# google-research/simclr

Measured on AMD Instinct MI355X. Metric: images/sec (whole node), ResNet-50 1x SimCLR pretraining step @224px, higher is better.
Workload: dtype f32; 1 GPU; ResNet-50 1x, 224x224, 2 views/image, per-GPU batch 512, global batch 512, NT-Xent T=0.1 + linear-eval head + LARS, global BN, dp1; global_batch=512, parallelism=dp1

## Files before the change

### simclr_amd/csrc/conv.hip

```cpp
#include "common.h"
#include <stdlib.h>
#include <string.h>
#include <mutex>
#include <type_traits>

namespace {

enum { MODE_FWD = 0, MODE_DGRAD = 1 };

struct ConvP {
  const void* x;
  const void* w;
  void* y;
  float* stats;
  int V, IH, IW, IC, OH, OW, N, KH, KW, stride, pad;
  int pixpitch;
  int M, K;
  int nslot, accumulate;
  int m_tiles, n_tiles;
  int cs, py, px, cls_h, cls_w;
  int ntaps;
  int taps[9];
  unsigned long long tap_w, dy_w, dx_w;
  const void* bn_x;
// ... 364 lines not shown
#pragma unroll
        for (int o = 1; o < 16; o <<= 1) { s += __shfl_xor(s, o, 64); ss += __shfl_xor(ss, o, 64); }
        if (fl == 0) {
          const int nl = wn * 64 + ni * 16 + g * 4 + r;
          red[(wm * BN + nl) * 2] = s;
          red[(wm * BN + nl) * 2 + 1] = ss;
        }
      }
    }
    __syncthreads();
    if (tid < BN && n0 + tid < p.N) {
      float s = 0.f, ss = 0.f;
#pragma unroll
      for (int w = 0; w < WM; ++w) { s += red[(w * BN + tid) * 2]; ss += red[(w * BN + tid) * 2 + 1]; }
      float* st = p.stats + (long long)(mt % p.nslot) * 2 * p.N;
      atomicAdd(st + n0 + tid, s);
      atomicAdd(st + p.N + n0 + tid, ss);
    }
    __syncthreads();
  }

  if (LDS_EPI) {
    constexpr int PITCH = BN * 2 + 8;
    constexpr int LPR = BN * 2 / 8;
    unsigned char* Cs = smem;
    long long* rowoff = (long long*)(smem + BM * PITCH);
    if (tid < BM) rowoff[tid] = row_offset(m0 + tid);
#pragma unroll
    for (int ni = 0; ni < NI; ++ni) {
      const int nl = wn * 64 + ni * 16 + g * 4;
#pragma unroll
      for (int mi = 0; mi < MI; ++mi) {
        const int ml = wm * (MI * 16) + mi * 16 + fl;
        u32x2 pk;
        pk[0] = pack_bf16x2(acc[ni][mi][0], acc[ni][mi][1]);
        pk[1] = pack_bf16x2(acc[ni][mi][2], acc[ni][mi][3]);
        *(u32x2*)(Cs + ml * PITCH + nl * 2) = pk;
      }
    }
    __syncthreads();
    const int c8 = tid % LPR;
    const int ncol = n0 + c8 * 4;
#pragma unroll 4
    for (int r = tid / LPR; r < BM; r += 256 / LPR) {
      const long long off = rowoff[r];
      if (off >= 0 && ncol < p.N) {
        u32x2 v = *(const u32x2*)(Cs + r * PITCH + c8 * 8);
        uint16_t* dst = (uint16_t*)Y + off + ncol;
        if (p.accumulate) {
          const u32x2 o = *(const u32x2*)dst;
          v[0] = pack_bf16x2(__uint_as_float(v[0] << 16) + __uint_as_float(o[0] << 16),
                             __uint_as_float(v[0] & 0xffff0000u) + __uint_as_float(o[0] & 0xffff0000u));
          v[1] = pack_bf16x2(__uint_as_float(v[1] << 16) + __uint_as_float(o[1] << 16),
                             __uint_as_float(v[1] & 0xffff0000u) + __uint_as_float(o[1] & 0xffff0000u));
        }
        *(u32x2*)dst = v;
      }
    }
  } else {
#pragma unroll
    for (int mi = 0; mi < MI; ++mi) {
      const long long off = row_offset(m0 + wm * (MI * 16) + mi * 16 + fl);
#pragma unroll
      for (int ni = 0; ni < NI; ++ni) {
        const int n = n0 + wn * 64 + ni * 16 + g * 4;
        if (off >= 0 && n < p.N) {
          T* dst = Y + off + n;
          float v[4] = {acc[ni][mi][0], acc[ni][mi][1], acc[ni][mi][2], acc[ni][mi][3]};
          if (p.accumulate) {
#pragma unroll
            for (int r = 0; r < 4; ++r) v[r] += Elem<T>::ld(dst + r);
          }
          *(float4*)dst = make_float4(v[0], v[1], v[2], v[3]);
        }
      }
    }
  }
}

#ifndef SIMCLR_BN64_WPE
#define SIMCLR_BN64_WPE 3
#endif
template <typename T, int MODE, int BM, int BN, int NW, int STAGES, bool STATS, bool BNEPI, bool EXT = false,
          bool WIN = false, bool FAPPLY = false, int SPL = 0, bool TAIL = false, bool PSB = false, int FAS = 0, int EPS = 0, bool PSX = false>
__global__ __launch_bounds__(NW * 64, (NW == 8 || STAGES == 3) ? 1 : (BN == 64 && (sizeof(T) == 2 || SPL == 13 || (SPL == 3 && PSB))) ? SIMCLR_BN64_WPE : 2) void conv_igemm_persistent(const ConvP p) {
  static_assert(EPS == 0 || (BNEPI && EPS <= 4 && (sizeof(T) == 2 || (MODE == MODE_DGRAD && SPL == 3 && PSB && PSX && !EXT))), "EPS specialises the BNEPI epilogue");
  const int bnm = EPS ? (((EPS - 1) >> 1) ? 4 : 2) : p.bn_mode;
  const bool accu = EPS ? ((EPS - 1) & 1) != 0 : p.accumulate != 0;
  static_assert(FAS == 0 || FAPPLY, "FAS specialises the FAPPLY epilogue");
  const bool fa_res = FAS ? true : p.bn_x != nullptr;
  const bool fa_rbn = FAS ? FAS == 2 : p.bn_mean != nullptr;
  const bool fa_relu = FAS ? true : p.bn_mode != 0;
  const bool fa_mask = FAS ? true : p.bn_mask != nullptr;
  const bool fa_n32 = FAS ? true : (p.N & 31) == 0;
  static_assert(!PSB || ((SPL == 3 || SPL == 13) && sizeof(T) == 4), "pre-split weights: fp32 storage, three terms");
  static_assert(!PSX || ((SPL == 3 || SPL == 13) && sizeof(T) == 4), "pre-split gathered operand: fp32 storage, three terms");
  static_assert(SPL != 13 || PSB, "split-fp16 terms need the pre-split (scaled) weight planes");
  static_assert(!WIN || (STAGES == 2 && !EXT && NW == 4 && BM == 128 && !FAPPLY && (sizeof(T) == 2 || ((SPL == 3 || SPL == 13) && PSB))),
                "halo-window variant: 2 stages; bf16, or fp32 storage with three terms and pre-split weights");
  static_assert(!FAPPLY || (MODE == MODE_FWD && !STATS && !BNEPI && !EXT), "fused BN-apply epilogue: forward, no statistics");
  static_assert(SPL == 0 || sizeof(T) == 4, "split-bf16 terms: fp32 storage only");
  constexpr bool WPS = WIN && sizeof(T) == 4 && !PSX && (SPL == 3 || SPL == 13);
  constexpr int EPC = Elem<T>::EPC;
  constexpr int BK = 8 * EPC;
  constexpr int WN = BN / 64;
  constexpr int WM = NW / WN;
  constexpr int MI = BM / WM / 16;
  constexpr int NI = 4;
  constexpr int AJ = BM / (8 * NW);
  constexpr int BJ = BN / (8 * NW);
  static_assert(AJ >= 1 && BJ >= 1 && MI >= 1, "tile / wave configuration");
  extern __shared__ __attribute__((aligned(16))) unsigned char smem[];
  constexpr int STG = (BM + BN) * 8;
  u32x4* As = (u32x4*)smem;
  u32x4* Bs = As + BM * 8;
  u32x4* Wn = (u32x4*)smem;
  u32x4* Bw = (u32x4*)(smem + (WIN ? p.win_bytes : 0));
  float* bnp = WIN ? (float*)(Bw + 2 * BN * 8)
                   : (float*)(As + STAGES * STG);
  long long* rowoff = (long long*)(bnp + (4 + (EXT ? 1 : 0)) * BN);
  const int zrow = WIN ? (int)(((unsigned char*)(rowoff + BM) - smem) >> 7) : 0;
  constexpr bool WSUM = BM == 256;
  float2* wred = (float2*)(rowoff + BM);
  constexpr bool LDS_EPI = sizeof(T) == 2;
  constexpr int NTH = NW * 64;
  constexpr int CPR = BN / 8;
  constexpr int RPP = NTH / CPR;
  constexpr bool ROWSTATS = STATS && LDS_EPI && (BNEPI || BM == 256);
  constexpr int EH = (LDS_EPI && BM * BN * 2 > STG * 16) ? 2 : 1;
  constexpr int BMH = BM / EH;
  static_assert(!LDS_EPI || (BMH * BN * 2 <= STG * 16), "C (half) tile must fit in one stage");
  static_assert(EH == 1 || (WM % EH == 0 && !WIN), "half-tile epilogue: whole waves per half");
  typedef __attribute__((address_space(1))) const void* gptr_t;
  typedef __attribute__((address_space(3))) void* lptr_t;

  const int tid = threadIdx.x, lane = tid & 63;
  const int wave = __builtin_amdgcn_readfirstlane(tid >> 6);
  const int g = lane >> 4, fl = lane & 15;
  const int wm = wave / WN, wn = wave % WN;
  const T* __restrict__ X = (const T*)p.x;
  const T* __restrict__ Wt = (const T*)p.w;
  T* __restrict__ Y = (T*)p.y;
  const int cls_hw = p.cls_h * p.cls_w;

  const int xcd = blockIdx.x & 7, l = blockIdx.x >> 3;
  const int nt = l % p.n_tiles;
  const int mslots = gridDim.x / p.n_tiles;
  const int mslot = (l / p.n_tiles) * 8 + xcd;
  const int n0 = nt * BN;
  const int count = (TAIL && p.rem_parts >= 2) ? p.rem_full : ((mslot < p.m_tiles) ? (p.m_tiles - mslot + mslots - 1) / mslots : 0);
  const bool has_part = TAIL && p.rem_parts >= 2 && mslot < p.rem_tiles * p.rem_parts;
  auto part_tile = [&]() __attribute__((always_inline)) { return p.rem_full * mslots + mslot / p.rem_parts; };
  auto part_index = [&]() __attribute__((always_inline)) { return mslot % p.rem_parts; };
  const int kpt = p.IC / BK;
  const int kpt2 = EXT ? p.ic2 / BK : 0;
  const int KT = p.ntaps * kpt + kpt2;
  const int kmain = p.KH * p.KW * p.IC;
  const T* __restrict__ X2 = (const T*)p.x2;

  const int kc = (lane & 7) ^ (lane >> 3);
  const bool flat = WIN || (p.KH == 1 && p.KW == 1 && p.stride == 1 && p.pad == 0 && p.cs == 1 &&
                            p.IH == p.OH && p.IW == p.OW);
  int a_ry[AJ], a_rx[AJ];
  int a_m[AJ];
  const T* a_rb[AJ];
  bool a_ok[AJ];
  const T* a_tp[AJ];
// ... 61 lines not shown
      __builtin_amdgcn_global_load_lds((gptr_t)src, (lptr_t)(b_dst + j * 1024), 16, 0, 0);
    }
  };

  if (BNEPI || EXT || FAPPLY) {
    for (int i = tid; i < BN; i += NW * 64) {
      const int n = n0 + i;
      const bool ok = n < p.N;
      if (FAPPLY) {
        bnp[i] = ok ? p.bn_scale[n] : 0.f;
        bnp[BN + i] = ok ? p.bn_shift[n] : 0.f;
        bnp[2 * BN + i] = (ok && p.bn_mean) ? p.bn_mean[n] : 1.f;
        bnp[3 * BN + i] = (ok && p.bn_rstd) ? p.bn_rstd[n] : 0.f;
      }
      if (BNEPI) {
        bnp[i] = (ok && bnm == 2) ? p.bn_scale[n] : 0.f;
        bnp[BN + i] = (ok && bnm == 2) ? p.bn_shift[n] : 0.f;
        bnp[2 * BN + i] = (ok && p.bn_mean) ? p.bn_mean[n] : 0.f;
        bnp[3 * BN + i] = (ok && p.bn_rstd) ? p.bn_rstd[n] : 0.f;
      }
      if (EXT) bnp[4 * BN + i] = (ok && p.bias) ? p.bias[n] : 0.f;
    }
  }
  if (WSUM && STATS && LDS_EPI) {
    for (int i = lane; i < BN; i += 64) wred[wave * BN + i] = make_float2(0.f, 0.f);
  }
  const int e_cc = tid % CPR;
  float e_s[8], e_q[8];
#pragma unroll
  for (int e = 0; e < 8; ++e) { e_s[e] = 0.f; e_q[e] = 0.f; }
  float st_s[NI][4], st_q[NI][4];
  if (STATS) {
#pragma unroll
    for (int i = 0; i < NI; ++i)
#pragma unroll
      for (int r = 0; r < 4; ++r) { st_s[i][r] = 0.f; st_q[i][r] = 0.f; }
  }

  int it = 0, iti = 0, ici = 0, ibuf = 0, buf = 0;
  int issued = 0, consumed = 0;
  const int KU = WIN ? kpt : KT;
  auto part_begin = [&]() __attribute__((always_inline)) { return (part_index() * KU) / p.rem_parts; };
  auto part_end = [&]() __attribute__((always_inline)) { return ((part_index() + 1) * KU) / p.rem_parts; };
  const int part_units = has_part ? part_end() - part_begin() : 0;
  const int total = WIN ? (count * kpt + part_units) * 9 : count * KT + part_units;
  auto issue_next = [&]() __attribute__((always_inline)) {
    issue_tile(iti, ici, ibuf);
    ibuf = (ibuf + 1 == STAGES) ? 0 : ibuf + 1;
    ++issued;
    if (++ici == ((EXT && iti == p.ntaps) ? kpt2 : kpt)) {
      ici = 0;
      if (++iti == p.ntaps + ((EXT && kpt2 > 0) ? 1 : 0)) {
        iti = 0;
        ++it;
        if (it < count) setup_rows(mslot + it * mslots);
        else if (it == count && has_part) {
          setup_rows(part_tile());
          const int pka = part_begin();
          iti = pka / kpt; ici = pka - iti * kpt;
          if (EXT && iti > p.ntaps) { iti = p.ntaps; ici = pka - p.ntaps * kpt; }
        }
      }
      if (it < count + (has_part ? 1 : 0) && iti < p.ntaps) set_tap(iti);
    }
  };
  const int Wd = p.IW;
  int wti = 0, wci = (WIN && count == 0 && has_part) ? part_begin() : 0, wit = 0;
  auto issue_b = [&]() __attribute__((always_inline)) {
    const int k0 = (int)((p.tap_w >> (4 * wti)) & 15) * p.IC + wci * BK;
    unsigned char* b_dst = (unsigned char*)(Bw + ibuf * (BN * 8)) + wave * BJ * 1024;
#pragma unroll
    for (int j = 0; j < BJ; ++j) {
      const void* src = b_ok[j] ? (const void*)(b_src[j] + k0) : p.zero;
      __builtin_amdgcn_global_load_lds((gptr_t)src, (lptr_t)(b_dst + j * 1024), 16, 0, 0);
    }
    ibuf ^= 1;
    ++issued;
    if (++wti == 9) {
      wti = 0;
      if (++wci == kpt) { wci = 0; if (++wit == count && has_part) wci = part_begin(); }
    }
  };
  auto issue_win = [&](int m0w, int c) __attribute__((always_inline)) {
    for (int j = 0; j < p.win_j; ++j) {
      const int blk = wave * p.win_j + j;
      const long long pix = (long long)m0w - (Wd + 1) + 8 * blk + (lane >> 3);
      const void* src = (pix >= 0 && pix < p.M) ? (const void*)(X + pix * p.pixpitch + c * BK + kc * EPC) : p.zero;
      __builtin_amdgcn_global_load_lds((gptr_t)src, (lptr_t)(smem + blk * 1024), 16, 0, 0);
    }
  };
  if (WIN) {
    if (tid < 8) Wn[zrow * 8 + tid] = zero16();
    if (total > 0) issue_b();
  } else if (total > 0) {
    if (count > 0) {
      setup_rows(mslot);
      set_tap(0);
    } else {
      setup_rows(part_tile());
      const int pka = part_begin();
      iti = pka / kpt; ici = pka - iti * kpt;
      if (EXT && iti > p.ntaps) { iti = p.ntaps; ici = pka - p.ntaps * kpt; }
      if (iti < p.ntaps) set_tap(iti);
    }
#pragma unroll
    for (int sidx = 0; sidx < STAGES - 1; ++sidx)
      if (issued < total) issue_next();
  }
  for (int ct = 0; ct < count + (has_part ? 1 : 0); ++ct) {
    const bool part = ct == count;
    const int m0 = (part ? part_tile() : mslot + ct * mslots) * BM;
    const int kt0 = part ? part_begin() : 0, kt1 = part ? part_end() : KU;
    f32x4 acc[NI][MI];
#pragma unroll
    for (int i = 0; i < NI; ++i)
#pragma unroll
      for (int j = 0; j < MI; ++j) acc[i][j] = (f32x4){0.f, 0.f, 0.f, 0.f};
    if (WIN) {
      const int m0w = m0;
      int rb[MI];
      unsigned vm[MI];
#pragma unroll
      for (int i = 0; i < MI; ++i) {
        const int ml = wm * (MI * 16) + i * 16 + fl;
        rb[i] = ml + Wd + 1;
        const int m = m0w + ml;
        unsigned msk = 0;
        if (m < p.M) {
          const int q = m / Wd, x = m - q * Wd, y = q % p.IH;
          const unsigned cm = (x > 0 ? 1u : 0u) | 2u | (x < Wd - 1 ? 4u : 0u);
          msk = (y > 0 ? cm : 0u) | (cm << 3) | (y < p.IH - 1 ? cm << 6 : 0u);
        }
        vm[i] = msk;
      }
      auto win_rows = [&](int t, int zr, int* rr) __attribute__((always_inline)) {
        const int ody = (int)((p.dy_w >> (4 * t)) & 15) - 8 - (MODE == MODE_FWD ? p.pad : 0);
        const int odx = (int)((p.dx_w >> (4 * t)) & 15) - 8 - (MODE == MODE_FWD ? p.pad : 0);
        const int doff = ody * Wd + odx, vbit = (ody + 1) * 3 + (odx + 1);
#pragma unroll
        for (int i = 0; i < MI; ++i) rr[i] = ((vm[i] >> vbit) & 1u) ? rb[i] + doff : zr;
      };
      auto win_load = [&](const u32x4* Wc, const int* rr, const u32x4* Bt, int ks, u32x4* af, u32x4* bf) __attribute__((always_inline)) {
#pragma unroll
        for (int i = 0; i < MI; ++i) af[i] = Wc[rr[i] * 8 + ((ks * 4 + g) ^ (rr[i] & 7))];
#pragma unroll
        for (int i = 0; i < NI; ++i) {
          const int r = wn * 64 + i * 16 + fl;
          bf[i] = Bt[r * 8 + ((ks * 4 + g) ^ (r & 7))];
        }
      };
      auto win_mma = [&](const u32x4* af, const u32x4* bf) __attribute__((always_inline)) {
#pragma unroll
        for (int ni = 0; ni < NI; ++ni)
#pragma unroll
          for (int mi = 0; mi < MI; ++mi) acc[ni][mi] = MMA<T>::run(bf[ni], af[mi], acc[ni][mi]);
      };
      auto win_step = [&](const u32x4* Wc, int zr, const u32x4* Bt, int t) __attribute__((always_inline)) {
        int rr[MI];
        win_rows(t, zr, rr);
        if constexpr (sizeof(T) == 4) {
          mma_f32_chunks<NI, MI, false, SPL, PSB, PSX || WPS>(&acc[0][0],
              [&](int i, int ks) { const int r = wn * 64 + i * 16 + fl; return Bt[r * 8 + ((ks * 4 + g) ^ (r & 7))]; },
              [&](int i, int ks) { return Wc[rr[i] * 8 + ((ks * 4 + g) ^ (rr[i] & 7))]; });
        } else {
#pragma unroll
        for (int ks = 0; ks < 2; ++ks) {
          u32x4 af[MI], bf[NI];
          win_load(Wc, rr, Bt, ks, af, bf);
          win_mma(af, bf);
        }
        }
      };
      for (int c = kt0; c < kt1; ++c) {
        __syncthreads();
        issue_win(m0w, c);
        for (int t = 0; t < 9; ++t) {
          asm volatile("s_waitcnt vmcnt(0)" ::: "memory");
          __syncthreads();
          if (issued < total) issue_b();
          if constexpr (WPS) {
            if (t == 0) {
              const int nq = p.win_j * 32 * 4;
              for (int q = tid; q < nq; q += NW * 64) {
                const int row = q >> 2, gq = q & 3;
                u32x4* w0 = Wn + row * 8 + (gq ^ (row & 7));
                u32x4* w1 = Wn + row * 8 + ((4 + gq) ^ (row & 7));
                u32x4 hi, lo;
                if constexpr (SPL == 13) split_terms2_f16(*w0, *w1, hi, lo); else split_terms2(*w0, *w1, hi, lo);
                *w0 = hi; *w1 = lo;
              }
              __syncthreads();
            }
          }
          win_step(Wn, zrow, Bw + buf * (BN * 8), t);
          buf ^= 1;
          ++consumed;
        }
      }
    } else
    for (int kt = kt0; kt < kt1; ++kt) {
      if (STAGES == 3 && issued - consumed >= 2) asm volatile("s_waitcnt vmcnt(%0)" ::"n"(AJ + BJ) : "memory");
      else asm volatile("s_waitcnt vmcnt(0)" ::: "memory");
      if (STAGES == 3) {
        asm volatile("s_waitcnt lgkmcnt(0)" ::: "memory");
        __builtin_amdgcn_s_barrier();
      } else {
        __syncthreads();
      }
      if (issued < total) issue_next();
      if constexpr (sizeof(T) == 4) {
        if (!DIAG(1))
          mma_f32_chunks<NI, MI, false, SPL, PSB, PSX>(&acc[0][0],
              [&](int i, int ks) { const int r = wn * 64 + i * 16 + fl; return Bs[buf * STG + r * 8 + ((ks * 4 + g) ^ (r & 7))]; },
              [&](int i, int ks) { const int r = wm * (MI * 16) + i * 16 + fl; return As[buf * STG + r * 8 + ((ks * 4 + g) ^ (r & 7))]; });
      } else
      if (!DIAG(1))
#pragma unroll
      for (int ks = 0; ks < 2; ++ks) {
        constexpr int MH = MI > 4 ? 4 : MI;
        u32x4 bf[NI];
#pragma unroll
        for (int i = 0; i < NI; ++i) {
          const int r = wn * 64 + i * 16 + fl;
          bf[i] = Bs[buf * STG + r * 8 + ((ks * 4 + g) ^ (r & 7))];
        }
#pragma unroll
        for (int mh = 0; mh < MI; mh += MH) {
          u32x4 af[MH];
#pragma unroll
          for (int i = 0; i < MH; ++i) {
            const int r = wm * (MI * 16) + (mh + i) * 16 + fl;
            af[i] = As[buf * STG + r * 8 + ((ks * 4 + g) ^ (r & 7))];
          }
#pragma unroll
          for (int ni = 0; ni < NI; ++ni)
#pragma unroll
            for (int mi = 0; mi < MH; ++mi) acc[ni][mh + mi] = MMA<T>::run(bf[ni], af[mi], acc[ni][mh + mi]);
        }
      }
      buf = (buf + 1 == STAGES) ? 0 : buf + 1;
      ++consumed;
    }
    if (DIAG(4)) {
      if (acc[0][0][0] == 12345.678f) Y[0] = (T)0;
      continue;
    }
    if constexpr (SPL == 13) {
#pragma unroll
      for (int i = 0; i < NI; ++i)
#pragma unroll
        for (int j = 0; j < MI; ++j) acc[i][j] *= (1.0f / (float)(1 << F16_WSCALE_LOG2));
    }
    if (part) {
      const long long slot0 = ((long long)(mslot / p.rem_parts) * p.n_tiles + nt) * (p.rem_parts - 1);
      const int pj = part_index();
      constexpr int FR = NI * MI;
      if (pj != 0) {
        const __amdgpu_buffer_rsrc_t rp = __builtin_amdgcn_make_buffer_rsrc(
            (void*)((f32x4*)p.part_ws + (slot0 + pj - 1) * (long long)(FR * NTH)), 0, FR * NTH * 16, 0x00020000);
#pragma unroll
        for (int ni = 0; ni < NI; ++ni)
#pragma unroll
          for (int mi = 0; mi < MI; ++mi)
            __builtin_amdgcn_raw_buffer_store_b128(__builtin_bit_cast(u32x4, acc[ni][mi]), rp, tid * 16, (ni * MI + mi) * NTH * 16, 16);
// ... 1985 lines not shown
  const long long nchunks = e[2] * 8;
  const bool f16 = e[3] != 0;
  for (long long i = blockIdx.x * 256ll + threadIdx.x; i < nchunks; i += (long long)gridDim.x * 256ll) {
    const long long blk = i >> 3;
    const int c = (int)(i & 7), gq = c & 3;
    u32x4 c0 = *(const u32x4*)(src + blk * 32 + gq * 4), c1 = *(const u32x4*)(src + blk * 32 + 16 + gq * 4);
    u32x4 hi, lo;
    if (f16) {
#pragma unroll
      for (int q = 0; q < 4; ++q) { c0[q] = __float_as_uint(__uint_as_float(c0[q]) * f16_scale); c1[q] = __float_as_uint(__uint_as_float(c1[q]) * f16_scale); }
      split_terms2_f16(c0, c1, hi, lo);
    } else {
      split_terms2(c0, c1, hi, lo);
    }
    *(u32x4*)(dst + i * 4) = (c < 4) ? hi : lo;
  }
}

__global__ __launch_bounds__(256) void presplit_packed(const float4* __restrict__ src, u32x4* __restrict__ dst, long long npix) {
  for (long long i = blockIdx.x * 256ll + threadIdx.x; i < npix; i += (long long)gridDim.x * 256ll) {
    const float4 v = src[i];
    uint32_t h0, l0, h1, l1;
    split_pair<false>(v.x, v.y, h0, l0);
    split_pair<false>(v.z, v.w, h1, l1);
    dst[i] = (u32x4){h0, h1, l0, l1};
  }
}

__global__ void unpack_stem_dw(const float* __restrict__ src, float* __restrict__ dst, int KH, int KW,
                               int CI, int CO, int KWP, int accumulate) {
  const int total = KH * KW * CI * CO;
  for (int i = blockIdx.x * blockDim.x + threadIdx.x; i < total; i += gridDim.x * blockDim.x) {
    const int co = i % CO;
    const int ci = (i / CO) % CI;
    const int kw = (i / (CO * CI)) % KW;
    const int kh = i / (CO * CI * KW);
    const float v = src[(long long)((kh * KWP + kw) * 4 + ci) * CO + co];
    dst[i] = accumulate ? dst[i] + v : v;
  }
}

static int g_f32_terms_fwd = 0, g_f32_terms_bwd = 0;
static bool valid_terms(int t, bool fwd) { return t == 0 || t == 3 || t == 6 || (fwd && t == 13); }
static int terms_of(int* dtype, bool fwd) {
  const int f = (*dtype >> 12) & 0xff;
  *dtype &= ~(0xff << 12);
  if (f == 0) return fwd ? g_f32_terms_fwd : g_f32_terms_bwd;
  return valid_terms(f - 1, fwd) ? f - 1 : -1;
}

static bool take_ps_w(int* dtype) {
  const bool f = (*dtype & SIMCLR_FMT_PS_W) != 0;
  *dtype &= ~SIMCLR_FMT_PS_W;
  return f;
}

static thread_local char g_last_inst[512] = "";
static bool dry_run() { return simclr_dry_run(); }
template <typename T, int MODE> static void record_inst(const char* kern, unsigned grid, unsigned block, size_t lds, const ConvP& p) {
  snprintf(g_last_inst, sizeof(g_last_inst), "(%s) elt=%d role=%s grid=%u block=%u lds=%zu m_tiles=%d n_tiles=%d tail_parts=%d", kern,
           (int)sizeof(T), MODE == MODE_FWD ? "fwd" : "dgrad", grid, block, lds, p.m_tiles, p.n_tiles, p.rem_parts);
}
template <typename T> static const char* type_name() { return sizeof(T) == 2 ? "uint16_t" : "float"; }
static const char* mode_name(int mode) { return mode == MODE_FWD ? "MODE_FWD" : "MODE_DGRAD"; }
static const char* tf(bool v) { return v ? "true" : "false"; }

template <typename T, int MODE, int BN, bool STATS, bool GLDS>
static void run_igemm(dim3 grid, dim3 block, size_t lds, hipStream_t stream, const ConvP& p) {
  char name[128];
  snprintf(name, sizeof(name), "conv_igemm<%s, %s, %d, %s, %s>", type_name<T>(), mode_name(MODE), BN, tf(STATS), tf(GLDS));
  record_inst<T, MODE>(name, grid.x, block.x, lds, p);
  if (!dry_run()) hipLaunchKernelGGL((conv_igemm<T, MODE, BN, STATS, GLDS>), grid, block, lds, stream, p);
}

template <int MODE, bool STATS, bool BNEPI, bool FLAT>
static void run_wide(dim3 grid, dim3 block, size_t lds, hipStream_t stream, const ConvP& p) {
  char name[128];
  snprintf(name, sizeof(name), "conv_igemm_wide<%s, %s, %s, %s>", mode_name(MODE), tf(STATS), tf(BNEPI), tf(FLAT));
  record_inst<uint16_t, MODE>(name, grid.x, block.x, lds, p);
  if (!dry_run()) hipLaunchKernelGGL((conv_igemm_wide<MODE, STATS, BNEPI, FLAT>), grid, block, lds, stream, p);
}

template <typename T, int MODE, int BM, int BN, int NW, int STAGES, bool STATS, bool BNEPI, bool EXT = false,
          bool WIN = false, bool FAPPLY = false, int SPL = 0, bool TAIL = false, bool PSB = false, int FAS = 0, int EPS = 0, bool PSX = false>
static void run_persistent(dim3 grid, dim3 block, size_t lds, hipStream_t stream, const ConvP& p) {
  const int opt[9] = {EXT, WIN, FAPPLY, SPL, TAIL, PSB, FAS, EPS, PSX};
  const bool is_bool[9] = {true, true, true, false, true, true, false, false, true};
  int n = 9;
  while (n > 0 && opt[n - 1] == 0) --n;
  char name[256];
  int len = snprintf(name, sizeof(name), "conv_igemm_persistent<%s, %s, %d, %d, %d, %d, %s, %s", type_name<T>(), mode_name(MODE), BM, BN, NW,
                     STAGES, tf(STATS), tf(BNEPI));
  for (int i = 0; i < n; ++i)
    len += is_bool[i] ? snprintf(name + len, sizeof(name) - len, ", %s", tf(opt[i])) : snprintf(name + len, sizeof(name) - len, ", %d", opt[i]);
  snprintf(name + len, sizeof(name) - len, ">");
  record_inst<T, MODE>(name, grid.x, block.x, lds, p);
  if (!dry_run())
    hipLaunchKernelGGL((conv_igemm_persistent<T, MODE, BM, BN, NW, STAGES, STATS, BNEPI, EXT, WIN, FAPPLY, SPL, TAIL, PSB, FAS, EPS, PSX>),
                       grid, block, lds, stream, p);
}

template <int KPT, int FAS>
static void run_nwalk(dim3 grid, dim3 block, size_t lds, hipStream_t stream, const ConvP& p) {
  char name[64];
  snprintf(name, sizeof(name), "conv_igemm_nwalk<%d, %d>", KPT, FAS);
  record_inst<float, MODE_FWD>(name, grid.x, block.x, lds, p);
  const size_t len = strlen(g_last_inst);
  snprintf(g_last_inst + len, sizeof(g_last_inst) - len, " walk=n_inner n_group=%d n_groups=%d", p.nw_gw, p.nw_groups);
  if (!dry_run()) hipLaunchKernelGGL((conv_igemm_nwalk<KPT, FAS>), grid, block, lds, stream, p);
}

struct WgradRec { int k_tiles, n_tiles, splits, chunks_per_split, xcd_map; };
static WgradRec rec_of(const WgradP& p) { return {p.k_tiles, p.n_tiles, p.splits, p.chunks_per_split, p.xcd_map}; }
static WgradRec rec_of(const Wgrad3P& p) { return {p.ci_tiles, p.co_tiles, p.splits, p.chunks_per_split, 1}; }
static WgradRec rec_of(const StemWgP& p) { return {1, 1, p.splits, p.chunks_per_split, 0}; }
static void record_wgrad(const char* kern, int elt, const char* role, unsigned grid, unsigned block, size_t lds, const WgradRec& r) {
  snprintf(g_last_inst, sizeof(g_last_inst), "(%s) elt=%d role=%s grid=%u block=%u lds=%zu k_tiles=%d n_tiles=%d splits=%d chunks_per_split=%d xcd_map=%d",
           kern, elt, role, grid, block, lds, r.k_tiles, r.n_tiles, r.splits, r.chunks_per_split, r.xcd_map);
}

template <typename T, int BKW, int BNW, bool MT = false>
static void run_wgrad(const char* role, unsigned grid, unsigned block, size_t lds, hipStream_t stream, const WgradP& p) {
  char name[128];
  snprintf(name, sizeof(name), MT ? "conv_wgrad<%s, %d, %d, true>" : "conv_wgrad<%s, %d, %d>", type_name<T>(), BKW, BNW);
  record_wgrad(name, (int)sizeof(T), role, grid, block, lds, rec_of(p));
  if (!dry_run()) hipLaunchKernelGGL((conv_wgrad<T, BKW, BNW, MT>), dim3(grid), dim3(block), lds, stream, p);
}

template <typename T, int BKW, int BNW, int BRM, int STAGES, int WK = 2, int WNN = 2, bool GRAM = false, bool MT = false, int SPL = 0, int PSD = 0>
static void run_wgrad_dma(const char* role, unsigned grid, unsigned block, size_t lds, hipStream_t stream, const WgradP& p) {
  const int opt[6] = {WK, WNN, GRAM, MT, SPL, PSD}, dflt[6] = {2, 2, 0, 0, 0, 0};
  const bool is_bool[6] = {false, false, true, true, false, false};
  int n = 6;
  while (n > 0 && opt[n - 1] == dflt[n - 1]) --n;
  char name[160];
  int len = snprintf(name, sizeof(name), "conv_wgrad_dma<%s, %d, %d, %d, %d", type_name<T>(), BKW, BNW, BRM, STAGES);
  for (int i = 0; i < n; ++i)
    len += is_bool[i] ? snprintf(name + len, sizeof(name) - len, ", %s", tf(opt[i])) : snprintf(name + len, sizeof(name) - len, ", %d", opt[i]);
  snprintf(name + len, sizeof(name) - len, ">");
  record_wgrad(name, (int)sizeof(T), role, grid, block, lds, rec_of(p));
  if (!dry_run())
    hipLaunchKernelGGL((conv_wgrad_dma<T, BKW, BNW, BRM, STAGES, WK, WNN, GRAM, MT, SPL, PSD>), dim3(grid), dim3(block), lds, stream, p);
}

template <int ST> static void run_wgrad3x3_bf16(unsigned grid, unsigned block, size_t lds, hipStream_t stream, const Wgrad3P& q) {
  char name[64];
  snprintf(name, sizeof(name), "conv_wgrad3x3_bf16<%d>", ST);
  record_wgrad(name, 2, "wgrad", grid, block, lds, rec_of(q));
  if (!dry_run()) hipLaunchKernelGGL(conv_wgrad3x3_bf16<ST>, dim3(grid), dim3(block), lds, stream, q);
}
static void run_wgrad3x3_f32ps(unsigned grid, unsigned block, size_t lds, hipStream_t stream, const Wgrad3P& q) {
  record_wgrad("conv_wgrad3x3_f32ps", 4, "wgrad", grid, block, lds, rec_of(q));
  if (!dry_run()) hipLaunchKernelGGL(conv_wgrad3x3_f32ps, dim3(grid), dim3(block), lds, stream, q);
}
template <int STAGES> static void run_stem_wgrad_ps(unsigned grid, unsigned block, size_t lds, hipStream_t stream, const StemWgP& p) {
  char name[64];
  snprintf(name, sizeof(name), "stem_wgrad_ps<7, 2, %d>", STAGES);
  record_wgrad(name, 4, "stem_wgrad_ps", grid, block, lds, rec_of(p));
  if (!dry_run()) hipLaunchKernelGGL((stem_wgrad_ps<7, 2, STAGES>), dim3(grid), dim3(block), lds, stream, p);
}
static void run_slab_reduce(const void* slabs, int splits, long long numel, float* out, int accumulate, hipStream_t stream) {
  const int grid = max(1, (int)ceil_div(numel / 4, 16));
  const size_t len = strlen(g_last_inst);
  snprintf(g_last_inst + len, sizeof(g_last_inst) - len, " reduce_grid=%d", grid);
  if (!dry_run()) hipLaunchKernelGGL(slab_reduce, dim3(grid), dim3(256), 0, stream, (const float*)slabs, splits, numel, out, accumulate);
}

static const void* zero_page() {
  static void* zp = nullptr;
  if (dry_run()) return (const void*)&g_last_inst;
  if (!zp && hipGetSymbolAddress(&zp, HIP_SYMBOL(g_zero16)) != hipSuccess) zp = nullptr;
  return zp;
}

static void igemm_persistent_grid(long long M, int N, int* bn, int* n_tiles, int* grid, bool narrow = false) {
  const int BN = (N <= 64 || narrow) ? 64 : 128;
  const int m_tiles = (int)((M + 127) / 128);
  const int nt = ceil_div(N, BN);
  const int unit = 8 * nt;
  const int resident = (BN == 64 ? 3 : 2) * 256;
  int pg = (resident / unit) * unit;
// ... 98 lines not shown
        (lost && hipMemcpyAsync(sc->flags + want_n, &lost, sizeof(unsigned), hipMemcpyHostToDevice, stream) != hipSuccess) ||
        (lost && hipStreamSynchronize(stream) != hipSuccess)) {
      (void)hipGetLastError();
      if (sc->ws) (void)hipFree(sc->ws);
      if (sc->flags) (void)hipFree(sc->flags);
      sc->ws = nullptr; sc->flags = nullptr;
      return false;
    }
    sc->floats = want_f; sc->nflags = want_n;
  }
  p.part_ws = sc->ws; p.part_flags = sc->flags; p.part_err = sc->flags + sc->nflags;
  return true;
}

static int split_tail_timeouts(unsigned* host_total) {
  SIMCLR_CHECK_ARG(host_total != nullptr, "conv2d_split_tail_timeouts: null argument");
  std::lock_guard<std::mutex> lock(g_scratch_mutex);
  unsigned total = 0;
  for (int i = 0; i < g_split_scratch_n; ++i) {
    if (!g_split_scratch[i].flags) continue;
    unsigned v = 0;
    if (hipMemcpy(&v, g_split_scratch[i].flags + g_split_scratch[i].nflags, sizeof(unsigned), hipMemcpyDeviceToHost) != hipSuccess) {
      simclr_set_error("conv2d_split_tail_timeouts: %s", hipGetErrorString(hipGetLastError()));
      return 2;
    }
    total += v;
    if (v != 0 && hipMemset(g_split_scratch[i].flags, 0, g_split_scratch[i].nflags * sizeof(unsigned)) != hipSuccess) {
      simclr_set_error("conv2d_split_tail_timeouts: %s", hipGetErrorString(hipGetLastError()));
      return 2;
    }
  }
  *host_total = total;
  return 0;
}

struct PresplitScratch { hipStream_t stream; void* buf; size_t bytes; };
static PresplitScratch g_presplit[8];
static int g_presplit_n = 0;
static thread_local int g_last_presplit = 0;
static bool presplit_enabled(long long rows, int K) {
  const char* e = getenv("SIMCLR_F32_PRESPLIT");
  return !(e && atoi(e) == 0) && K % 32 == 0 && rows > 0;
}
static const void* presplit_weights(const void* w, long long rows, int K, hipStream_t stream, bool f16) {
  if (dry_run()) return w;
  std::lock_guard<std::mutex> lock(g_scratch_mutex);
  PresplitScratch* sc = nullptr;
  for (int i = 0; i < g_presplit_n; ++i)
    if (g_presplit[i].stream == stream) sc = &g_presplit[i];
  if (!sc) {
    if (g_presplit_n == 8) return nullptr;
    sc = &g_presplit[g_presplit_n++];
    *sc = PresplitScratch{stream, nullptr, 0};
  }
  const size_t need = (size_t)rows * K * sizeof(float);
  if (sc->bytes < need) {
    if (sc->buf) (void)hipFree(sc->buf);
    sc->buf = nullptr; sc->bytes = 0;
    const size_t want = need < (16u << 20) ? (16u << 20) : need;
    if (hipMalloc(&sc->buf, want) != hipSuccess) { (void)hipGetLastError(); sc->buf = nullptr; return nullptr; }
    sc->bytes = want;
  }
  const long long nblocks = rows * (K / 32);
  if (f16) hipLaunchKernelGGL(presplit_rows<true>, dim3((unsigned)ceil_div(nblocks * 8, 256)), dim3(256), 0, stream,
                              (const float*)w, (uint32_t*)sc->buf, nblocks, (float)(1 << F16_WSCALE_LOG2));
  else hipLaunchKernelGGL(presplit_rows<false>, dim3((unsigned)ceil_div(nblocks * 8, 256)), dim3(256), 0, stream,
                          (const float*)w, (uint32_t*)sc->buf, nblocks, 1.0f);
  return sc->buf;
}

struct IgemmPlan {
  enum Family {
    EMPTY,
    UNSUPPORTED,
    WIDE,
    TILE256,
    TILE128,
    NWALK,
    FALLBACK,
  } family = EMPTY;
  ConvP p;
  int bn = 0, spl = 0, fas = 0, eps = 0;
  bool stats = false, bnepi = false, ext = false, win = false, fapply = false, tail = false, psb = false, psx = false;
  bool flat = false;
  unsigned grid = 0, block = 0;
  size_t lds = 0;
  size_t tile_floats = 0;
  bool presplit = false;
};

static bool igemm_nwalk_on() {
  const char* e = getenv("SIMCLR_IGEMM_NWALK");
  return !e || atoi(e) != 0;
}

static void plan_nwalk(IgemmPlan& k) {
  ConvP& p = k.p;
  const bool flat = p.KH == 1 && p.KW == 1 && p.stride == 1 && p.pad == 0 && p.cs == 1 && p.IH == p.OH && p.IW == p.OW;
  if (!igemm_nwalk_on() || !flat || !k.fapply || !k.psb || k.spl != 13 || k.psx || p.x2 || (p.IC != 64 && p.IC != 128) || p.K != p.IC ||
      p.pixpitch < p.IC || (p.pixpitch & 3) || (p.N & 63) || p.N <= 128 || p.N > 512 || !p.bn_x || !p.bn_mode || !p.bn_mask ||
      ((uintptr_t)p.bn_mask & 15) || p.rem_parts >= 2)
    return;
  const int m_tiles = ceil_div(p.M, 64);
  int groups = 1;
  while (m_tiles * groups < 2 * 3 * 256 && (p.N / groups) % 128 == 0) groups *= 2;
  const int gw = p.N / groups;
  const size_t lds = (size_t)(p.IC / 32) * 64 * 128 + 2 * 64 * 128 + (p.bn_mean ? 4 : 2) * gw * sizeof(float);
  const int per_cu = 3 * lds <= 160 * 1024 ? 3 : 2;
  const int unit = 8 * groups;
  int pg = max(unit, (per_cu * 256 / unit) * unit);
  const int need = ceil_div(m_tiles, 8) * unit;
  if (pg > need) pg = need;
  k.family = IgemmPlan::NWALK;
  k.bn = 64; k.fas = p.bn_mean ? 2 : 1;
  k.grid = pg; k.block = 256; k.lds = lds;
  p.m_tiles = m_tiles; p.n_tiles = p.N / 64;
  p.nw_groups = groups; p.nw_gw = gw;
}

template <typename T, int MODE>
static IgemmPlan plan_igemm(const ConvP& p0, bool can_split, bool can_presplit) {
  constexpr bool bf16 = sizeof(T) == 2, fwd = MODE == MODE_FWD;
  IgemmPlan k;
  ConvP& p = k.p;
  p = p0;
  const bool narrow = igemm_narrow(p, sizeof(T), !fwd);
  const int BN = (p.N <= 64 || narrow) ? 64 : 128;
  p.m_tiles = ceil_div(p.M, 128);
  p.n_tiles = ceil_div(p.N, BN);
  if (p.M <= 0) return k;
#ifdef SIMCLR_DIAG
  { const char* e = getenv("SIMCLR_DIAG"); p.diag = e ? atoi(e) : 0; }
#endif
  const bool st = p.stats != nullptr;
  k.bnepi = p.bn_mode != 0;
  k.ext = p.x2 != nullptr;
  k.stats = k.bnepi || (st && !k.ext);
  const bool odd_n = bf16 && (p.N & 7) != 0;
  if (p.ntaps <= 0 || p.n_tiles > 64 || odd_n) {
    if (p.x_ps || (p.w_ps && p.ntaps > 0) || p.accumulate == 2) { k.family = IgemmPlan::UNSUPPORTED; return k; }
    if ((odd_n && (p.bn_mode || p.fapply || p.x2)) || !p.y) { k.family = IgemmPlan::UNSUPPORTED; return k; }
    k.family = IgemmPlan::FALLBACK;
    k.bn = BN; k.stats = st; k.bnepi = k.ext = false;
    k.grid = ceil_div(p.m_tiles, 8) * 8 * p.n_tiles; k.block = 256;
    k.lds = 2 * (128 + BN) * 128;
    const size_t epi = 128 * (BN * 2 + 8) + 128 * sizeof(long long);
    if (bf16 && epi > k.lds) k.lds = epi;
    return k;
  }
  const bool wide = bf16 && igemm_use_wide(p, fwd);
  if (wide || (bf16 && igemm_use_256(p, fwd))) {
    p.m_tiles = ceil_div(p.M, 256);
    p.n_tiles = p.N / 256;
    const int unit = 8 * p.n_tiles;
    k.grid = min(max(unit, (256 / unit) * unit), ceil_div(p.m_tiles, 8) * unit);
    k.block = 512;
    k.tile_floats = (size_t)256 * 256;
    if (wide) {
      k.family = IgemmPlan::WIDE;
      p.x_bytes = (unsigned)((long long)p.V * p.IH * p.IW * p.pixpitch * 2);
      const int dist[3] = {8, 128, 136}, chw = p.cls_h * p.cls_w;
      for (int i = 0; i < 3; ++i) {
        p.rs_dq[i] = dist[i] / chw;
        const int r = dist[i] - p.rs_dq[i] * chw;
        p.rs_drow[i] = r / p.cls_w; p.rs_dcol[i] = r - p.rs_drow[i] * p.cls_w;
      }
      k.lds = 131072 + 4 * 256 * sizeof(float) + 256 * sizeof(long long) + 8 * 256 * 2 * sizeof(float) + 4 * 512 * sizeof(int);
      if (can_split) split_tail_plan(p, k.grid, p.ntaps * (p.IC / 64), 1, true);
      k.flat = p.KH == 1 && p.KW == 1 && p.stride == 1 && p.pad == 0 && p.cs == 1 && p.IH == p.OH && p.IW == p.OW;
    } else {
      k.family = IgemmPlan::TILE256;
      k.bn = 256;
      k.lds = 2 * (256 + 256) * 128 + 5 * 256 * sizeof(float) + 256 * sizeof(long long) + 8 * 256 * 2 * sizeof(float);
      k.fapply = p.fapply != 0;
      if (k.fapply) k.stats = k.bnepi = k.ext = false;
      else if (can_split) split_tail_plan(p, k.grid, p.ntaps * (p.IC / 64) + (p.x2 ? p.ic2 / 64 : 0), 1);
      k.tail = p.rem_parts >= 2;
    }
    return k;
  }
  k.family = IgemmPlan::TILE128;
  k.bn = BN;
  int pg, bn_, nt_;
  igemm_persistent_grid(p.M, p.N, &bn_, &nt_, &pg, narrow);
  k.grid = pg; k.block = 256;
  k.lds = 2 * (128 + BN) * 128 + 5 * BN * sizeof(float) + 128 * sizeof(long long);
  const bool win3 = (bf16 || p.split == 3 || p.split == 13) && !p.fapply && !p.x2 && p.KH == 3 && p.KW == 3 && p.stride == 1 &&
                    p.pad == 1 && p.cs == 1 && p.ntaps == 9 && p.IH == p.OH && p.IW == p.OW && p.IW <= 62 && p.accumulate < 2;
  const int bk_elems = 128 / (int)sizeof(T);
  if (bf16 && BN == 128 && !p.fapply && can_split) {
    split_tail_plan(p, pg, win3 ? p.IC / bk_elems : p.ntaps * (p.IC / bk_elems) + (p.x2 ? p.ic2 / bk_elems : 0), win3 ? 9 : 1);
    k.tile_floats = (size_t)128 * BN;
  } else {
    p.rem_parts = 0;
  }
  k.tail = p.rem_parts >= 2;
  if (!bf16) {
    const bool presplit = can_presplit && presplit_enabled(p.N, p.K);
    if (!fwd && p.split == 3) { k.psb = true; k.presplit = !p.w_ps && presplit; }
    if (fwd && p.split == 13) { k.psb = true; k.presplit = !p.w_ps && presplit; }
    if (k.psb && !p.w_ps && !presplit) {
      k.psb = false;
      if (fwd) p.split = 6;
    }
    if ((p.x_ps && !k.psb) || (p.w_ps && !k.psb)) { k.family = IgemmPlan::UNSUPPORTED; return k; }
    k.spl = k.psb || p.split == 3 || p.split == 6 ? p.split : 0;
    k.psx = k.psb && p.x_ps;
  }
  if (p.fapply) {
    k.fapply = true;
    k.stats = k.bnepi = k.ext = false;
    if (bf16 && p.bn_x && p.bn_mode && p.bn_mask && (p.N & 31) == 0) k.fas = p.bn_mean ? 2 : 1;
    if (!bf16 && fwd) plan_nwalk(k);
    return k;
  }
  int eps = 0;
  if (bf16 && !fwd && p.bn_mode && !k.tail) {
    if (p.bn_mode == 2 && !p.accumulate) eps = 1;
    else if (p.bn_mode == 4) eps = p.accumulate ? 4 : 3;
  }
  k.win = bf16 ? win3 : win3 && k.psb && (fwd ? !p.bn_mode : p.x_ps && (p.bn_mode != 0) == st);
  if (!bf16 && !fwd && k.psb && k.spl == 3 && k.psx && !k.ext && (p.bn_mode == 2 || p.bn_mode == 4) && p.accumulate < 2 && (p.N & 63) == 0 &&
      ((uintptr_t)p.bn_mask & 15) == 0 && f32_eps_exists(k.win, 1 + (p.bn_mode == 4 ? 2 : 0) + p.accumulate) && f32_epi_batch())
    eps = 1 + (p.bn_mode == 4 ? 2 : 0) + p.accumulate;
  if (k.win) {
    const int rows = ((128 + 2 * (p.IW + 1)) + 31) / 32 * 32;
    p.win_j = rows / 32;
    p.win_bytes = (!bf16 || rows * 128 > 128 * BN * 2) ? rows * 128 : 128 * BN * 2;
    k.lds = (size_t)p.win_bytes + 2 * BN * 128 + 5 * BN * sizeof(float) + 128 * sizeof(long long) + 128;
    k.eps = (!bf16 || eps == 1) ? eps : 0;
  } else {
    k.eps = !bf16 || eps == 1 || (!k.ext && eps >= 3) ? eps : 0;
    if (k.psx && k.ext) k.family = IgemmPlan::UNSUPPORTED;
  }
  return k;
}

template <typename V, V... Vs> struct among {};
template <typename F> static bool with_consts(F&& f) { return f(); }
template <typename V, V... Vs, typename... Rest, typename F>
static bool with_consts(F&& f, among<V, Vs...>, V x, Rest... rest) {
  bool hit = false;
  (void)((x == Vs && (hit = with_consts([&](auto... c) { return f(std::integral_constant<V, Vs>{}, c...); }, rest...), true)) || ...);
  return hit;
}
using Bools = among<bool, false, true>;

static constexpr bool epilogue_exists(bool st, bool be, bool ex) { return (st || !be) && (!ex || st == be); }
static constexpr bool tile128_exists(bool bf16, bool fwd, int bn, bool st, bool be, bool ex, bool win, bool fa, int spl, bool tail,
                                     bool psb, int fas, int eps, bool psx) {
  if (fa)
    return fwd && !st && !be && !ex && !win && !tail && !eps && !psx && (bf16 ? spl == 0 && !psb : fas == 0 && psb == (spl == 13));
  if (fas || !epilogue_exists(st, be, ex) || (win && ex)) return false;
  if (bf16)
    return spl == 0 && !psb && !psx && (eps ? st && be && !tail && (eps == 1 || (!ex && !win && (eps == 3 || eps == 4))) : !tail || bn == 128);
  if (tail) return false;
  if (eps) return !fwd && st && be && psb && spl == 3 && !ex && psx && f32_eps_exists(win, eps);
  if (win) return psb && (fwd ? spl == 13 && !be && !psx : spl == 3 && psx);
  if (psx) return !fwd && !ex && psb && spl == 3;
  if (psb) return fwd ? spl == 13 && !be && !ex : spl == 3;
  return spl == 0 || spl == 3 || spl == 6;
}

template <typename T, int MODE>
static bool launch_plan(const IgemmPlan& k, hipStream_t s) {
  constexpr bool bf16 = sizeof(T) == 2, fwd = MODE == MODE_FWD;
  const dim3 g(k.grid), b(k.block);
  switch (k.family) {
    case IgemmPlan::FALLBACK:
      return with_consts([&](auto BN, auto ST) { run_igemm<T, MODE, BN, ST, true>(g, b, k.lds, s, k.p); return true; },
                         among<int, 64, 128>{}, k.bn, Bools{}, k.stats);
    case IgemmPlan::WIDE:
      if constexpr (bf16)
        return with_consts([&](auto ST, auto BE, auto FLAT) {
          if constexpr (!epilogue_exists(ST, BE, false)) return false;
          else { run_wide<MODE, ST, BE, FLAT>(g, b, k.lds, s, k.p); return true; }
        }, Bools{}, k.stats, Bools{}, k.bnepi, Bools{}, k.flat);
      return false;
    case IgemmPlan::TILE256:
      if constexpr (bf16)
        return with_consts([&](auto ST, auto BE, auto EX, auto FA, auto TAIL) {
          if constexpr (FA ? !(fwd && !ST && !BE && !EX && !TAIL) : !epilogue_exists(ST, BE, EX)) return false;
          else { run_persistent<T, MODE, 256, 256, 8, 2, ST, BE, EX, false, FA, 0, TAIL>(g, b, k.lds, s, k.p); return true; }
        }, Bools{}, k.stats, Bools{}, k.bnepi, Bools{}, k.ext, Bools{}, k.fapply, Bools{}, k.tail);
      return false;
    case IgemmPlan::TILE128: {
      using Spl = std::conditional_t<bf16, among<int, 0>, among<int, 0, 3, 6, 13>>;
      using FpBools = std::conditional_t<bf16, among<bool, false>, Bools>;
      using HBools = std::conditional_t<bf16, Bools, among<bool, false>>;
      using Fas = std::conditional_t<bf16, among<int, 0, 1, 2>, among<int, 0>>;
      using Eps = std::conditional_t<bf16, among<int, 0, 1, 3, 4>, among<int, 0>>;
      if constexpr (!bf16 && !fwd) {
        if (k.eps)
          return k.stats && k.bnepi && !k.ext && !k.win && !k.fapply && k.spl == 3 && !k.tail && k.psb && !k.fas && k.psx &&
                 with_consts([&](auto BN, auto EPS) {
                   static_assert(f32_eps_exists(false, EPS), "the list below = the epilogues f32_eps_exists names");
                   run_persistent<T, MODE, 128, BN, 4, 2, true, true, false, false, false, 3, false, true, 0, EPS, true>(g, b, k.lds, s, k.p);
                   return true;
                 }, among<int, 64, 128>{}, k.bn, among<int, 1, 4>{}, k.eps);
      }
      return with_consts([&](auto BN, auto ST, auto BE, auto EX, auto WIN, auto FA, auto SPL, auto TAIL, auto PSB, auto FAS, auto EPS, auto PSX) {
        if constexpr (!tile128_exists(bf16, fwd, BN, ST, BE, EX, WIN, FA, SPL, TAIL, PSB, FAS, EPS, PSX)) return false;
        else { run_persistent<T, MODE, 128, BN, 4, 2, ST, BE, EX, WIN, FA, SPL, TAIL, PSB, FAS, EPS, PSX>(g, b, k.lds, s, k.p); return true; }
      }, among<int, 64, 128>{}, k.bn, Bools{}, k.stats, Bools{}, k.bnepi, Bools{}, k.ext, Bools{}, k.win, Bools{}, k.fapply, Spl{}, k.spl,
         HBools{}, k.tail, FpBools{}, k.psb, Fas{}, k.fas, Eps{}, k.eps, FpBools{}, k.psx);
    }
    case IgemmPlan::NWALK:
      if constexpr (!bf16 && fwd)
        return with_consts([&](auto KPT, auto FAS) { run_nwalk<KPT, FAS>(g, b, k.lds, s, k.p); return true; },
                           among<int, 2, 4>{}, k.p.IC / 32, among<int, 1, 2>{}, k.fas);
      return false;
    default:
      return false;
  }
}

template <typename T, int MODE>
static int launch_igemm_one(const ConvP& p, hipStream_t stream) {
  bool can_split = true, can_presplit = true;
  IgemmPlan k = plan_igemm<T, MODE>(p, can_split, can_presplit);
  if (k.family == IgemmPlan::UNSUPPORTED) return 1;
  if (k.p.rem_parts >= 2 && !split_tail_scratch(k.p, k.tile_floats, stream)) k = plan_igemm<T, MODE>(p, can_split = false, can_presplit);
  if (k.presplit) {
    const void* ws = presplit_weights(k.p.w, k.p.N, k.p.K, stream, k.spl == 13);
    if (ws) k.p.w = ws;
    else k = plan_igemm<T, MODE>(p, can_split, can_presplit = false);
  }
  if (k.family == IgemmPlan::EMPTY) return 0;
  if (k.family == IgemmPlan::UNSUPPORTED) return 1;
  if (k.family != IgemmPlan::FALLBACK) g_last_split_parts = k.p.rem_parts;
  if (sizeof(T) == 4 && MODE == MODE_DGRAD && k.family == IgemmPlan::TILE128) g_last_presplit = k.psb;
  return launch_plan<T, MODE>(k, stream) ? 0 : 1;
}

template <typename T, int MODE>
static int launch_igemm(const ConvP& p0, hipStream_t stream) {
  ConvP p = p0;
  if (MODE == MODE_FWD || p.stride == 1) {
    p.cs = 1; p.py = 0; p.px = 0; p.cls_h = p.OH; p.cls_w = p.OW;
    p.ntaps = p.KH * p.KW;
    p.tap_w = p.dy_w = p.dx_w = 0;
    for (int t = 0; t < p.ntaps; ++t) {
      p.taps[t] = t;
      const int ty = t / p.KW, tx = t % p.KW;
      const int dy = (MODE == MODE_FWD) ? ty : p.pad - ty, dx = (MODE == MODE_FWD) ? tx : p.pad - tx;
      p.tap_w |= (unsigned long long)t << (4 * t);
      p.dy_w |= (unsigned long long)(dy + 8) << (4 * t);
      p.dx_w |= (unsigned long long)(dx + 8) << (4 * t);
    }
    p.M = p.V * p.OH * p.OW;
    return launch_igemm_one<T, MODE>(p, stream);
  }
  const int S = p.stride;
  ConvP cls[4];
  int n = 0;
  for (int py = 0; py < S; ++py)
    for (int px = 0; px < S; ++px) {
      ConvP q = p;
      q.cs = S; q.py = py; q.px = px;
      q.cls_h = (p.OH - py + S - 1) / S;
      q.cls_w = (p.OW - px + S - 1) / S;
      q.ntaps = 0;
      q.tap_w = q.dy_w = q.dx_w = 0;
      for (int ty = 0; ty < p.KH; ++ty)
        for (int tx = 0; tx < p.KW; ++tx)
          if ((py + p.pad - ty) % S == 0 && (px + p.pad - tx) % S == 0 && q.ntaps < 9) {
            q.tap_w |= (unsigned long long)(ty * p.KW + tx) << (4 * q.ntaps);
            q.dy_w |= (unsigned long long)((py + p.pad - ty) / S + 8) << (4 * q.ntaps);
            q.dx_w |= (unsigned long long)((px + p.pad - tx) / S + 8) << (4 * q.ntaps);
            q.taps[q.ntaps++] = ty * p.KW + tx;
          }
      q.M = p.V * q.cls_h * q.cls_w;
      if (q.ntaps == 0 && p.accumulate == 2 && ((py | px) & 1)) q.accumulate = 0;
      else if (q.ntaps == 0 && p.accumulate) continue;
      if (p.accumulate == 3) q.accumulate = 0;
      if (q.ntaps == 0) q.x_ps = 0;
      if (plan_igemm<T, MODE>(q, true, true).family == IgemmPlan::UNSUPPORTED) return 1;
      cls[n++] = q;
    }
  for (int i = 0; i < n; ++i)
    if (int rc = launch_igemm_one<T, MODE>(cls[i], stream)) return rc;
  return 0;
// ... 698 lines not shown
```

Measured before the change: 3794 images/s.

## Prefetch next halo window through registers during fp32 window conv taps

Adds a WPF variant of the fp32 halo-window forward conv kernel. It loads the next channel chunk's (or next tile's) input window into registers during tap 7 and writes it to LDS, with the hi/lo split applied, after the 9-tap loop. The old path issued window loads at the start of each chunk, waited for them, and split in place, so this change overlaps that latency with MMA work. In exchange it uses more VGPRs (3x2 u32x4 per thread), which may hurt occupancy, and it ties the variant to a narrow config set (BN=128, SPL=13, win_j<=6). It also adds DIAG hooks that skip window loading or splitting.

Result: no change. 3805 images/s, median of 6 (+0.3%).

```diff
diff --git a/simclr_amd/csrc/conv.hip b/simclr_amd/csrc/conv.hip
--- a/simclr_amd/csrc/conv.hip
+++ b/simclr_amd/csrc/conv.hip
@@ -470,7 +470,8 @@
 #define SIMCLR_BN64_WPE 3
 #endif
 template <typename T, int MODE, int BM, int BN, int NW, int STAGES, bool STATS, bool BNEPI, bool EXT = false,
-          bool WIN = false, bool FAPPLY = false, int SPL = 0, bool TAIL = false, bool PSB = false, int FAS = 0, int EPS = 0, bool PSX = false>
+          bool WIN = false, bool FAPPLY = false, int SPL = 0, bool TAIL = false, bool PSB = false, int FAS = 0, int EPS = 0, bool PSX = false,
+          bool WPF = false>
 __global__ __launch_bounds__(NW * 64, (NW == 8 || STAGES == 3) ? 1 : (BN == 64 && (sizeof(T) == 2 || SPL == 13 || (SPL == 3 && PSB))) ? SIMCLR_BN64_WPE : 2) void conv_igemm_persistent(const ConvP p) {
   static_assert(EPS == 0 || (BNEPI && EPS <= 4 && (sizeof(T) == 2 || (MODE == MODE_DGRAD && SPL == 3 && PSB && PSX && !EXT))), "EPS specialises the BNEPI epilogue");
   const int bnm = EPS ? (((EPS - 1) >> 1) ? 4 : 2) : p.bn_mode;
@@ -698,6 +699,7 @@
     }
   };
   auto issue_win = [&](int m0w, int c) __attribute__((always_inline)) {
+    if (DIAG(32)) return;
     for (int j = 0; j < p.win_j; ++j) {
       const int blk = wave * p.win_j + j;
       const long long pix = (long long)m0w - (Wd + 1) + 8 * blk + (lane >> 3);
@@ -705,9 +707,41 @@
       __builtin_amdgcn_global_load_lds((gptr_t)src, (lptr_t)(smem + blk * 1024), 16, 0, 0);
     }
   };
+  static_assert(!WPF || (WIN && sizeof(T) == 4 && !TAIL && BN == 128), "window prefetch: fp32 halo window on the 128 x 128 tile");
+  constexpr int PFJ = 3;
+  u32x4 sg[PFJ][2];
+  auto stage_load = [&](int j, int m0w, int c, bool live) __attribute__((always_inline)) {
+    const int q = tid + NTH * j, row = q >> 2, gq = q & 3;
+    const long long pix = (long long)m0w - (Wd + 1) + row;
+    const bool ok = live && row < p.win_j * 32 && pix >= 0 && pix < p.M;
+    const u32x4* s0 = ok ? (const u32x4*)(X + pix * p.pixpitch + c * BK) + gq : (const u32x4*)p.zero;
+    sg[j][0] = s0[0];
+    sg[j][1] = s0[ok ? 4 : 0];
+  };
+  auto stage_store = [&]() __attribute__((always_inline)) {
+#pragma unroll
+    for (int j = 0; j < PFJ; ++j) {
+      const int q = tid + NTH * j, row = q >> 2, gq = q & 3;
+      if (row < p.win_j * 32) {
+        u32x4 hi = sg[j][0], lo = sg[j][1];
+        if constexpr (WPS) {
+          if constexpr (SPL == 13) split_terms2_f16(sg[j][0], sg[j][1], hi, lo); else split_terms2(sg[j][0], sg[j][1], hi, lo);
+        }
+        Wn[row * 8 + (gq ^ (row & 7))] = hi;
+        Wn[row * 8 + ((4 + gq) ^ (row & 7))] = lo;
+      }
+    }
+  };
   if (WIN) {
     if (tid < 8) Wn[zrow * 8 + tid] = zero16();
     if (total > 0) issue_b();
+    if constexpr (WPF) {
+      if (total > 0) {
+#pragma unroll
+        for (int j = 0; j < PFJ; ++j) stage_load(j, mslot * BM, 0, true);
+        stage_store();
+      }
+    }
   } else if (total > 0) {
     if (count > 0) {
       setup_rows(mslot);
@@ -787,6 +821,36 @@
         }
         }
       };
+      if constexpr (WPF) {
+        for (int c = kt0; c < kt1; ++c) {
+          const bool last_c = c + 1 == kt1;
+          const bool live = !last_c || ct + 1 < count;
+          const int nm0 = last_c ? (mslot + (ct + 1) * mslots) * BM : m0w, nc = last_c ? 0 : c + 1;
+#pragma nounroll
+          for (int t = 0; t < 9; ++t) {
+            if (t == 8) asm volatile("s_waitcnt vmcnt(%0)" ::"n"(2 * PFJ) : "memory");
+            else asm volatile("s_waitcnt vmcnt(0)" ::: "memory");
+            asm volatile("s_waitcnt lgkmcnt(0)" ::: "memory");
+            __builtin_amdgcn_s_barrier();
+            asm volatile("" ::: "memory");
+            if (issued < total) issue_b();
+            asm volatile("" ::: "memory");
+            if (t == 7) {
+#pragma unroll
+              for (int j = 0; j < PFJ; ++j) stage_load(j, nm0, nc, live);
+              asm volatile("" ::: "memory");
+            }
+            win_step(Wn, zrow, Bw + buf * (BN * 8), t);
+            buf ^= 1;
+            ++consumed;
+          }
+          asm volatile("s_waitcnt vmcnt(0)" ::: "memory");
+          asm volatile("s_waitcnt lgkmcnt(0)" ::: "memory");
+          __builtin_amdgcn_s_barrier();
+          asm volatile("" ::: "memory");
+          if (live) stage_store();
+        }
+      } else
       for (int c = kt0; c < kt1; ++c) {
         __syncthreads();
         issue_win(m0w, c);
@@ -795,7 +859,7 @@
           __syncthreads();
           if (issued < total) issue_b();
           if constexpr (WPS) {
-            if (t == 0) {
+            if (t == 0 && !DIAG(64)) {
               const int nq = p.win_j * 32 * 4;
               for (int q = tid; q < nq; q += NW * 64) {
                 const int row = q >> 2, gq = q & 3;
@@ -2947,7 +3011,8 @@
 }
 
 template <typename T, int MODE, int BM, int BN, int NW, int STAGES, bool STATS, bool BNEPI, bool EXT = false,
-          bool WIN = false, bool FAPPLY = false, int SPL = 0, bool TAIL = false, bool PSB = false, int FAS = 0, int EPS = 0, bool PSX = false>
+          bool WIN = false, bool FAPPLY = false, int SPL = 0, bool TAIL = false, bool PSB = false, int FAS = 0, int EPS = 0, bool PSX = false,
+          bool WPF = false>
 static void run_persistent(dim3 grid, dim3 block, size_t lds, hipStream_t stream, const ConvP& p) {
   const int opt[9] = {EXT, WIN, FAPPLY, SPL, TAIL, PSB, FAS, EPS, PSX};
   const bool is_bool[9] = {true, true, true, false, true, true, false, false, true};
@@ -2960,8 +3025,12 @@
     len += is_bool[i] ? snprintf(name + len, sizeof(name) - len, ", %s", tf(opt[i])) : snprintf(name + len, sizeof(name) - len, ", %d", opt[i]);
   snprintf(name + len, sizeof(name) - len, ">");
   record_inst<T, MODE>(name, grid.x, block.x, lds, p);
+  if (WPF) {
+    const size_t rl = strlen(g_last_inst);
+    snprintf(g_last_inst + rl, sizeof(g_last_inst) - rl, " win_prefetch=1");
+  }
   if (!dry_run())
-    hipLaunchKernelGGL((conv_igemm_persistent<T, MODE, BM, BN, NW, STAGES, STATS, BNEPI, EXT, WIN, FAPPLY, SPL, TAIL, PSB, FAS, EPS, PSX>),
+    hipLaunchKernelGGL((conv_igemm_persistent<T, MODE, BM, BN, NW, STAGES, STATS, BNEPI, EXT, WIN, FAPPLY, SPL, TAIL, PSB, FAS, EPS, PSX, WPF>),
                        grid, block, lds, stream, p);
 }
 
@@ -3226,6 +3295,7 @@
   ConvP p;
   int bn = 0, spl = 0, fas = 0, eps = 0;
   bool stats = false, bnepi = false, ext = false, win = false, fapply = false, tail = false, psb = false, psx = false;
+  bool wpf = false;
   bool flat = false;
   unsigned grid = 0, block = 0;
   size_t lds = 0;
@@ -3235,6 +3305,11 @@
 
 static bool igemm_nwalk_on() {
   const char* e = getenv("SIMCLR_IGEMM_NWALK");
+  return !e || atoi(e) != 0;
+}
+
+static bool win_prefetch_on() {
+  const char* e = getenv("SIMCLR_WIN_PREFETCH");
   return !e || atoi(e) != 0;
 }
 
@@ -3373,6 +3448,7 @@
     p.win_bytes = (!bf16 || rows * 128 > 128 * BN * 2) ? rows * 128 : 128 * BN * 2;
     k.lds = (size_t)p.win_bytes + 2 * BN * 128 + 5 * BN * sizeof(float) + 128 * sizeof(long long) + 128;
     k.eps = (!bf16 || eps == 1) ? eps : 0;
+    k.wpf = !bf16 && fwd && BN == 128 && p.win_j <= 6 && win_prefetch_on();
   } else {
     k.eps = !bf16 || eps == 1 || (!k.ext && eps >= 3) ? eps : 0;
     if (k.psx && k.ext) k.family = IgemmPlan::UNSUPPORTED;
@@ -3442,6 +3518,14 @@
                    run_persistent<T, MODE, 128, BN, 4, 2, true, true, false, false, false, 3, false, true, 0, EPS, true>(g, b, k.lds, s, k.p);
                    return true;
                  }, among<int, 64, 128>{}, k.bn, among<int, 1, 4>{}, k.eps);
+      }
+      if constexpr (!bf16 && fwd) {
+        if (k.wpf)
+          return k.bn == 128 && !k.bnepi && !k.ext && k.win && !k.fapply && k.spl == 13 && !k.tail && k.psb && !k.fas && !k.eps && !k.psx &&
+                 with_consts([&](auto ST) {
+                   run_persistent<T, MODE, 128, 128, 4, 2, ST, false, false, true, false, 13, false, true, 0, 0, false, true>(g, b, k.lds, s, k.p);
+                   return true;
+                 }, Bools{}, k.stats);
       }
       return with_consts([&](auto BN, auto ST, auto BE, auto EX, auto WIN, auto FA, auto SPL, auto TAIL, auto PSB, auto FAS, auto EPS, auto PSX) {
         if constexpr (!tile128_exists(bf16, fwd, BN, ST, BE, EX, WIN, FA, SPL, TAIL, PSB, FAS, EPS, PSX)) return false;
```
